# hamorrar/juicefs

Hardware: AMD Instinct MI355X
Metric: sealed+checksummed GB/s, 4 MiB blocks (higher is better)
Workload: dtype u8; 1 GPU; 64.0 GiB device-resident batch of 4 MiB blocks per GPU, aes256gcm seal + CRC32C full; blocks_per_gpu=16384, resident_blocks_per_gpu=16384, block_bytes=4194304, algo=aes256gcm, mode=seal, aes_kernel=ttable, engine=one process per GPU, parallelism=block-sharded x1, no collective

## Files before the change

juicefs_amd/csrc/jfsx_gcm.hip:

```cpp

#include "jfsx_dev.h"

#define JFSX_HD __device__ __forceinline__
#define BS3(a, b, c, tt) __builtin_amdgcn_bitop3_b32((a), (b), (c), (tt))
#define PERM(hi, lo, sel) __builtin_amdgcn_perm((hi), (lo), (sel))
#define OPAQUE(x)                                 \
    do {                                          \
        (x) = __builtin_amdgcn_readfirstlane(x);  \
        asm volatile("" : "+s"(x));               \
    } while (0)
#include "jfsx_aes_bs.h"

namespace jfsx {

constexpr int kAeadNt = 3;
constexpr uint32_t kLdsCrc = 0;
constexpr uint32_t kLdsTT = 20480;
constexpr uint32_t kLdsGh = 24576;
constexpr uint32_t kLdsAesOff = 24576;
constexpr uint32_t kLdsAes = 65536 + kLdsAesOff;
constexpr uint32_t kLdsBasis = kLdsAes + 65536;
constexpr uint32_t kLdsSegRaw = kLdsBasis + 2048;
constexpr uint32_t kLdsSegFlag = kLdsSegRaw + 512;
constexpr uint32_t kLdsP = kLdsSegFlag + 512;
constexpr uint32_t kLdsBytes = kLdsP + 4096;

__device__ __forceinline__ uint32_t rotl8(uint32_t x) { return __builtin_amdgcn_alignbit(x, x, 24); }
__device__ __forceinline__ uint32_t xor3(uint32_t a, uint32_t b, uint32_t c) {
    return __builtin_amdgcn_bitop3_b32(a, b, c, 0x96);
}
__device__ __forceinline__ uint32_t rk_load(const uint32_t *rk, int i) {
    uint32_t k = rk[i];
    if (i >= 8 && i < 56) {
        k = (k >> 8) | (k << 24);
        OPAQUE(k);
    }
    return k;
}

#define AES_SEL(k) (0x0c020000u | ((4u + (k)) << 8))
#define TA(w, k) lds_u32(lds, __builtin_amdgcn_perm((w), loff, AES_SEL(k)) + kLdsAesOff)
#define TB(w, k) lds_u32(lds, __builtin_amdgcn_perm((w), loff, AES_SEL(k)) + (kLdsAesOff + 128u))

#define AES_COL(o, i0, i1, i2, i3, rkv) \
    o = xor3(TA(i0, 0), TB(i2, 2), rotl8(xor3(TA(i1, 1), TB(i3, 3), (rkv))));
#define AES_ROUND(o0, o1, o2, o3, i0, i1, i2, i3, r) \
    AES_COL(o0, i0, i1, i2, i3, rk[4 * (r) + 0])     \
    AES_COL(o1, i1, i2, i3, i0, rk[4 * (r) + 1])     \
    AES_COL(o2, i2, i3, i0, i1, rk[4 * (r) + 2])     \
    AES_COL(o3, i3, i0, i1, i2, rk[4 * (r) + 3])

#define AES_LAST(o, a, b, c, d, rkv)                                                             \
    o = __builtin_amdgcn_bitop3_b32(                                                             \
            __builtin_amdgcn_bitop3_b32(TB(a, 0), TA(b, 1), 0xffu, 0xe4) ,       \
            __builtin_amdgcn_bitop3_b32(TA(c, 2), TB(d, 3), 0x00ff0000u, 0xe4),                 \
            0x0000ffffu, 0xe4) ^ (rkv);

template <int NS>
__device__ __forceinline__ void aes_ctr_blocks(const char *lds, uint32_t loff, const uint32_t *rk, const uint32_t *k1,
                                               const uint32_t (&ctr)[NS], uint32_t (&ks)[NS][4]) {
    uint32_t a[NS][4], b[NS][4];
#pragma unroll
    for (int s = 0; s < NS; s++) {
        const uint32_t x3 = __builtin_bswap32(ctr[s]) ^ rk[3];
        a[s][0] = k1[0] ^ rotl8(TB(x3, 3));
        a[s][1] = k1[1] ^ TB(x3, 2);
        a[s][2] = k1[2] ^ rotl8(TA(x3, 1));
        a[s][3] = k1[3] ^ TA(x3, 0);
    }
#pragma unroll
    for (int r = 2; r <= 13; r += 2) {
#pragma unroll
        for (int s = 0; s < NS; s++) { AES_ROUND(b[s][0], b[s][1], b[s][2], b[s][3], a[s][0], a[s][1], a[s][2], a[s][3], r); }
#pragma unroll
        for (int s = 0; s < NS; s++) { AES_ROUND(a[s][0], a[s][1], a[s][2], a[s][3], b[s][0], b[s][1], b[s][2], b[s][3], r + 1); }
    }
#pragma unroll
    for (int s = 0; s < NS; s++) {
        AES_LAST(ks[s][0], a[s][0], a[s][1], a[s][2], a[s][3], rk[56]);
        AES_LAST(ks[s][1], a[s][1], a[s][2], a[s][3], a[s][0], rk[57]);
        AES_LAST(ks[s][2], a[s][2], a[s][3], a[s][0], a[s][1], rk[58]);
        AES_LAST(ks[s][3], a[s][3], a[s][0], a[s][1], a[s][2], rk[59]);
    }
}

__device__ __forceinline__ void aes_r2_uniform(const char *lds, uint32_t loff, const uint32_t *rk, const uint32_t *k1,
                                               uint32_t U, uint32_t (&u)[4]) {
    const uint32_t x3 = __builtin_bswap32(U << 8) ^ rk[3];
    const uint32_t a1 = k1[1] ^ TB(x3, 2);
    const uint32_t a2 = k1[2] ^ rotl8(TA(x3, 1));
    const uint32_t a3 = k1[3] ^ TA(x3, 0);
    u[0] = xor3(TB(a2, 2), rotl8(xor3(TA(a1, 1), TB(a3, 3), rk[8])), 0u);
    u[1] = xor3(TA(a1, 0), TB(a3, 2), rotl8(TA(a2, 1) ^ rk[9]));
    u[2] = xor3(TA(a2, 0), rotl8(xor3(TA(a3, 1), TB(a1, 3), rk[10])), 0u);
    u[3] = xor3(TA(a3, 0), TB(a1, 2), rotl8(TB(a2, 3) ^ rk[11]));
}

__device__ __forceinline__ uint4 aes_r2_entry(const char *lds, uint32_t loff, uint32_t rk3, uint32_t k10, uint32_t c) {
    const uint32_t x3 = (c << 24) ^ rk3;
    const uint32_t a0 = k10 ^ rotl8(TB(x3, 3));
    return make_uint4(TA(a0, 0), rotl8(TB(a0, 3)), TB(a0, 2), rotl8(TA(a0, 1)));
}

template <int I>
struct AesStep {
    static constexpr int value = I;
};
struct AesNoSide {
    template <int I>
    __device__ __forceinline__ void operator()(AesStep<I>) const {}
};
template <int NS, class Side = AesNoSide>
__device__ __forceinline__ void aes_ctr_blocks_u(const char *lds, uint32_t loff, const uint32_t *rk,
                                                 const uint32_t *k1, const uint32_t (&ctr)[NS],
                                                 const uint32_t (&u)[NS][4], const uint32_t (&du)[NS][4],
                                                 const uint32_t (&cym)[NS], uint32_t (&ks)[NS][4],
                                                 const Side &side = Side()) {
    uint32_t a[NS][4], b[NS][4];
#define UC(t, w) (__builtin_amdgcn_bitop3_b32((t), cym[s], du[s][w], 0x78) ^ u[s][w])
#pragma unroll
    for (int s = 0; s < NS; s++) {
        const uint4 pe = lds_u4(lds, ((ctr[s] << 4) & 0xff0u) + kLdsP);
        b[s][0] = UC(pe.x, 0);
        b[s][1] = UC(pe.y, 1);
        b[s][2] = UC(pe.z, 2);
        b[s][3] = UC(pe.w, 3);
    }
#undef UC
    side(AesStep<0>());
#pragma unroll
    for (int s = 0; s < NS; s++) { AES_ROUND(a[s][0], a[s][1], a[s][2], a[s][3], b[s][0], b[s][1], b[s][2], b[s][3], 3); }
    side(AesStep<1>());
#define JFSX_AES_PAIR(r)                                                                                                \
    _Pragma("unroll") for (int s = 0; s < NS; s++) {                                                                    \
        AES_ROUND(b[s][0], b[s][1], b[s][2], b[s][3], a[s][0], a[s][1], a[s][2], a[s][3], r);                           \
    }                                                                                                                   \
    side(AesStep<(r) - 2>());                                                                                           \
    _Pragma("unroll") for (int s = 0; s < NS; s++) {                                                                    \
        AES_ROUND(a[s][0], a[s][1], a[s][2], a[s][3], b[s][0], b[s][1], b[s][2], b[s][3], (r) + 1);                     \
    }                                                                                                                   \
    side(AesStep<(r) - 1>());
    JFSX_AES_PAIR(4)
    JFSX_AES_PAIR(6)
    JFSX_AES_PAIR(8)
    JFSX_AES_PAIR(10)
    JFSX_AES_PAIR(12)
#undef JFSX_AES_PAIR
#pragma unroll
    for (int s = 0; s < NS; s++) {
        AES_LAST(ks[s][0], a[s][0], a[s][1], a[s][2], a[s][3], 0u);
        AES_LAST(ks[s][1], a[s][1], a[s][2], a[s][3], a[s][0], 0u);
        AES_LAST(ks[s][2], a[s][2], a[s][3], a[s][0], a[s][1], 0u);
        AES_LAST(ks[s][3], a[s][3], a[s][0], a[s][1], a[s][2], 0u);
    }
}

struct GhLane {
    uint32_t sel[4];
    uint32_t off[4];
    bool r1, r2;
    uint32_t p1, p2;
};

__device__ __forceinline__ GhLane gh_lane(uint32_t lane) {
    GhLane g;
    const uint32_t q = lane & 15, k = q >> 2;
#pragma unroll
    for (int bb = 0; bb < 4; bb++) g.sel[bb] = 0x0c0c0000u | ((4u + ((bb + q) & 3)) << 8) | (uint32_t)bb;
#pragma unroll
    for (int dd = 0; dd < 4; dd++) {
        uint32_t o = 0;
#pragma unroll
        for (int bb = 0; bb < 4; bb++) {
            const uint32_t j = 4 * ((dd + k) & 3) + ((bb + q) & 3);
            o |= (j << 4) << (8 * bb);
        }
        g.off[dd] = o;
    }
    g.r1 = (k & 1) != 0;
    g.r2 = (k & 2) != 0;
    g.p1 = g.r1 ? 0x07060504u : 0x03020100u;
    g.p2 = g.r2 ? 0x07060504u : 0x03020100u;
    return g;
}

__device__ __forceinline__ void gh_rho(const uint32_t a[4], const GhLane &g, uint32_t R[4]) {
    uint32_t u[4];
#pragma unroll
    for (int i = 0; i < 4; i++) u[i] = PERM(a[(i + 2) & 3], a[i], g.p2);
#pragma unroll
    for (int i = 0; i < 4; i++) R[i] = PERM(u[(i + 1) & 3], u[i], g.p1);
}
__device__ __forceinline__ void gh_rho_inv(const uint32_t R[4], const GhLane &g, uint32_t a[4]) {
    uint32_t u[4];
#pragma unroll
    for (int i = 0; i < 4; i++) u[i] = g.r1 ? R[(i + 3) & 3] : R[i];
#pragma unroll
    for (int i = 0; i < 4; i++) a[i] = g.r2 ? u[(i + 2) & 3] : u[i];
}

__device__ __forceinline__ void ghash_step(const char *lds, uint32_t R[4], const GhLane &g, uint4 c) {
#if JFSX_GH8 == 4
    uint32_t S[4] = {c.x, c.y, c.z, c.w};
#pragma unroll
    for (int h = 0; h < 4; h++) {
        uint4 t[4];
#pragma unroll
        for (int q = 0; q < 4; q++) t[q] = lds_u4(lds, kLdsGh + __builtin_amdgcn_perm(R[h], g.off[h], g.sel[q]));
#define GX(f, i) S[i] = xor3(xor3(t[0].f, t[1].f, t[2].f), t[3].f, S[i])
        GX(x, 0); GX(y, 1); GX(z, 2); GX(w, 3);
#undef GX
        __builtin_amdgcn_sched_barrier(0);
    }
#elif JFSX_GH8
    uint32_t S[4] = {c.x, c.y, c.z, c.w};
#pragma unroll
    for (int h = 0; h < 2; h++) {
        uint4 t[8];
#pragma unroll
        for (int q = 0; q < 8; q++) {
            const int dd = 2 * h + (q >> 2), bb = q & 3;
            t[q] = lds_u4(lds, kLdsGh + __builtin_amdgcn_perm(R[dd], g.off[dd], g.sel[bb]));
        }
#define GX(f, i) S[i] = xor3(xor3(t[0].f, t[1].f, t[2].f), xor3(t[3].f, t[4].f, t[5].f), xor3(t[6].f, t[7].f, S[i]))
        GX(x, 0); GX(y, 1); GX(z, 2); GX(w, 3);
#undef GX
        __builtin_amdgcn_sched_barrier(0);
    }
#else
    uint4 t[16];
#pragma unroll
    for (int dd = 0; dd < 4; dd++)
#pragma unroll
        for (int bb = 0; bb < 4; bb++)
            t[4 * dd + bb] = lds_u4(lds, kLdsGh + __builtin_amdgcn_perm(R[dd], g.off[dd], g.sel[bb]));
#define GX(f, cf) xor3(xor3(xor3(t[0].f, t[1].f, t[2].f), xor3(t[3].f, t[4].f, t[5].f), xor3(t[6].f, t[7].f, t[8].f)), \
                       xor3(t[9].f, t[10].f, t[11].f), xor3(xor3(t[12].f, t[13].f, t[14].f), t[15].f, cf))
    const uint32_t S[4] = {GX(x, c.x), GX(y, c.y), GX(z, c.z), GX(w, c.w)};
#undef GX
#endif
    gh_rho(S, g, R);
}

struct Stream {
    uint64_t sub0, sub1;
    uint32_t acc[4];
    uint64_t jlast;
    bool has;
    uint32_t A, lend;
    uint64_t seg0;
};

__device__ __forceinline__ void crc_share(char *lds, uint32_t slot, uint32_t raw) {
    atomicXor(reinterpret_cast<uint32_t *>(lds + kLdsSegRaw) + slot, raw);
    reinterpret_cast<uint32_t *>(lds + kLdsSegFlag)[slot] = 1u;
}

template <int CRCMODE>
__device__ __forceinline__ void crc_segment_done(const BlkDev &blk, const DevTables &tab, uint32_t lane, uint32_t xl,
                                                 uint64_t seg0, uint32_t A, bool partial, char *lds, uint64_t c0) {
    const uint32_t raw = wave_xor(crc_mulmod(xl, A));
    if (lane == 0) {
        if (partial) {
            crc_share(lds, (uint32_t)((seg0 - c0) / kSeg), raw);
            return;
        }
        const uint32_t crc = ~(tab.crcx[96] ^ raw);
        const uint64_t si = seg0 / kSeg;
        if ((CRCMODE & 3) == 1)
            *reinterpret_cast<uint32_t *>(blk.crc + 4 * si) = __builtin_bswap32(crc);
        else
            blk.crc_calc[si] = crc;
    }
}

template <int CRCMODE>
__device__ __noinline__ void crc_segment_end(const BlkDev &blk, const DevTables &tab, uint32_t lane, uint32_t xl,
                                             uint64_t seg0, uint64_t seg1, uint32_t A, uint32_t lend,
                                             uint64_t tailRef, bool partial, char *lds, uint32_t slot) {
    const uint32_t Lseg = (uint32_t)(seg1 - seg0);
    uint32_t v;
    if (lend == 0) {
        const uint32_t sh = tailRef == seg1 ? xl : crc_mulmod(crc_xpow8_fast((uint32_t)(seg1 - tailRef), tab.crcx), xl);
        v = crc_mulmod(sh, A);
    } else {
        v = crc_mulmod(crc_xpow8_fast(Lseg - lend, tab.crcx), A);
    }
    const uint32_t raw = wave_xor(v);
    if (lane == 0) {
        if (partial) {
            crc_share(lds, slot, raw);
            return;
        }
        const uint32_t K = Lseg == (uint32_t)kSeg ? tab.crcx[96] : crc_mulmod(crc_xpow8_fast(Lseg, tab.crcx), 0xffffffffu);
        const uint32_t crc = ~(K ^ raw);
        const uint64_t si = seg0 / kSeg;
        if ((CRCMODE & 3) == 1)
            *reinterpret_cast<uint32_t *>(blk.crc + 4 * si) = __builtin_bswap32(crc);
        else
            blk.crc_calc[si] = crc;
    }
}

template <bool OPEN, int CRCMODE>
__device__ __noinline__ Stream row_generic(char *lds, uint32_t loff, const GhLane gl, const GcmSched *sch,
                                           const BlkDev blk, const DevTables tab, uint32_t lane, uint32_t xl, Stream st,
                                           uint64_t row, uint64_t c0, uint64_t c1) {
    uint32_t rk[60];
#pragma unroll
    for (int i = 0; i < 60; i++) rk[i] = rk_load(sch->rk, i);
    const uint32_t k1[4] = {sch->k1[0], sch->k1[1], sch->k1[2], sch->k1[3]};
    const uint64_t o = row + 16 * lane;
    const uint64_t end = st.sub1;
    const bool valid = o < end, full = o + 16 <= end;
    uint4 d = load_piece(blk.src, o, end);
    const uint32_t ctr[1] = {(uint32_t)((o >> 4) + 2)};
    uint32_t ks[1][4];
    aes_ctr_blocks<1>(lds, loff, rk, k1, ctr, ks);
    uint4 x = make_uint4(d.x ^ ks[0][0], d.y ^ ks[0][1], d.z ^ ks[0][2], d.w ^ ks[0][3]);
    uint4 c = OPEN ? d : x, p = OPEN ? x : d;
    if (!full) {
        const int nv = valid ? (int)(end - o) : 0;
        uint32_t m[4];
        for (int k = 0; k < 4; k++) {
            int bytes = nv - 4 * k;
            m[k] = bytes >= 4 ? 0xffffffffu : (bytes <= 0 ? 0u : ((1u << (8 * bytes)) - 1u));
        }
        c.x &= m[0]; c.y &= m[1]; c.z &= m[2]; c.w &= m[3];
        p.x &= m[0]; p.y &= m[1]; p.z &= m[2]; p.w &= m[3];
    }
    if (valid) store_piece(blk.dst, o, end, OPEN ? p : c);
    uint32_t t[4] = {st.acc[0], st.acc[1], st.acc[2], st.acc[3]};
    ghash_step(lds, t, gl, c);
    if (valid) {
        st.acc[0] = t[0]; st.acc[1] = t[1]; st.acc[2] = t[2]; st.acc[3] = t[3];
        st.jlast = o >> 4;
        st.has = true;
    }
    const uint4 cq = crc_src<CRCMODE>(c, p);
    if (CRCMODE) {
        if (full) {
            st.A = crc_piece<kLdsCrc>(lds, st.A, cq.x, cq.y, cq.z, cq.w);
            st.lend = (uint32_t)(o + 16 - st.seg0);
        } else if (valid) {
            const uint32_t pw[4] = {cq.x, cq.y, cq.z, cq.w};
            st.A = crc_partial<kLdsCrc>(lds, st.A, pw, (int)(end - o));
            st.lend = (uint32_t)(end - st.seg0);
        }
        const uint64_t seg1 = st.seg0 + kSeg < c1 ? st.seg0 + kSeg : c1;
        if (row + 1024 >= seg1) {
            crc_segment_end<CRCMODE>(blk, tab, lane, xl, st.seg0, seg1, st.A, st.lend, row, st.seg0 < st.sub0, lds,
                                     (uint32_t)((st.seg0 - c0) / kSeg));
            st.A = 0;
            st.lend = 0;
            st.seg0 = seg1;
        }
    }
    return st;
}

template <bool BS>
struct GcmShape {
    static constexpr uint32_t waves = BS ? 8u : (uint32_t)kWaves;
    static constexpr uint32_t threads = waves * 64u;
};

#ifdef JFSX_KS_PHASES
__device__ unsigned long long g_main_ts[8];
#define MAIN_STAMP(cond, i)                                                                  \
    do {                                                                                     \
        __syncthreads();                                                                     \
        if ((cond) && threadIdx.x == 0) g_main_ts[i] = __builtin_amdgcn_s_memrealtime(); \
    } while (0)
#else
#define MAIN_STAMP(cond, i) ((void)0)
#endif

#ifdef JFSX_ABLATE_TRACE
__device__ uint64_t g_wgtrace[4 * 65536];
#endif

template <bool OPEN, int CRCMODE, bool BS, int KL1>
__device__ __forceinline__ void gcm_task(char *lds, const Task task, const BlkDev *__restrict__ blks,
                                         const GcmSched *__restrict__ sched, uint32_t *__restrict__ partial,
                                         uint32_t *__restrict__ pexp, const DevTables &tab, uint32_t tid,
                                         uint32_t wave, uint32_t lane, uint32_t loff, const GhLane &gl, uint32_t xl) {
#ifdef JFSX_ABLATE_TRACE
    const uint64_t trace_t0 = __builtin_amdgcn_s_memrealtime();
#endif
    const BlkDev blk = blks[task.blk];
    const GcmSched *sch = sched + task.blk;
    if (tid < 128)
        reinterpret_cast<uint4 *>(lds + kLdsBasis)[tid] = reinterpret_cast<const uint4 *>(sch->basis)[tid];
    if (tid < 256) reinterpret_cast<uint32_t *>(lds + kLdsSegRaw)[tid] = 0u;
    if (wave < 4) {
        uint32_t c = (wave << 6) | lane;
        asm volatile("" : "+v"(c));
        reinterpret_cast<uint4 *>(lds + kLdsP)[c] = aes_r2_entry(lds, loff, sch->rk[3], sch->k1[0], c);
    }
    __syncthreads();
    {
        uint4 *lg = reinterpret_cast<uint4 *>(lds + kLdsGh);
        const uint4 *lb = reinterpret_cast<const uint4 *>(lds + kLdsBasis);
#ifdef JFSX_ABLATE_GHBUILD
        if (false)
#endif
        for (uint32_t u = tid; u < 1024; u += GcmShape<BS>::threads) {
            const uint32_t j = u & 15, blow = u >> 4;
            uint4 z = make_uint4(0, 0, 0, 0);
#pragma unroll
            for (int k = 2; k < 8; k++) {
                if ((blow >> (7 - k)) & 1) {
                    const uint4 v = lb[8 * j + k];
                    z.x ^= v.x; z.y ^= v.y; z.z ^= v.z; z.w ^= v.w;
                }
            }
            const uint4 h0 = lb[8 * j], h1 = lb[8 * j + 1];
            lg[(blow << 4) | j] = z;
            lg[((blow | 64) << 4) | j] = make_uint4(z.x ^ h1.x, z.y ^ h1.y, z.z ^ h1.z, z.w ^ h1.w);
            lg[((blow | 128) << 4) | j] = make_uint4(z.x ^ h0.x, z.y ^ h0.y, z.z ^ h0.z, z.w ^ h0.w);
            lg[((blow | 192) << 4) | j] =
                make_uint4(z.x ^ h0.x ^ h1.x, z.y ^ h0.y ^ h1.y, z.z ^ h0.z ^ h1.z, z.w ^ h0.w ^ h1.w);
        }
    }
    __syncthreads();

    const bool first_task = task.blk == 0 && task.c0 == 0;
    MAIN_STAMP(first_task, 2);
    const uint64_t c0 = task.c0, c1 = task.c1;
    const uint32_t nseg = (uint32_t)((c1 - c0 + kSeg - 1) / kSeg);
    constexpr uint32_t V = GcmShape<BS>::waves;

    constexpr bool kRowSplit = !BS;
    Stream st;
    if (kRowSplit) {
        const uint32_t npairs = (uint32_t)((c1 - c0 + 2047) / 2048);
        const uint32_t ra = 2 * (wave * npairs / V), rb = 2 * ((wave + 1) * npairs / V);
        st.sub0 = c0 + (uint64_t)ra * 1024;
        st.sub1 = rb > ra ? (c0 + (uint64_t)rb * 1024 < c1 ? c0 + (uint64_t)rb * 1024 : c1) : st.sub0;
    } else {
        const uint32_t sa = wave * nseg / V, sb = (wave + 1) * nseg / V;
        st.sub0 = c0 + (uint64_t)sa * kSeg;
        st.sub1 = sb > sa ? (c0 + (uint64_t)sb * kSeg < c1 ? c0 + (uint64_t)sb * kSeg : c1) : st.sub0;
    }
    st.acc[0] = st.acc[1] = st.acc[2] = st.acc[3] = 0;
    st.jlast = 0;
    st.has = false;
    st.A = 0;
    st.lend = 0;
    st.seg0 = c0 + (st.sub0 - c0) / kSeg * kSeg;
    const bool act = st.sub1 > st.sub0;
    const uint64_t fr = (st.sub1 - st.sub0) / 1024;
    const uint64_t rf = act ? fr : 0;
    const uint64_t ld0 = st.sub0;
    const uint8_t *src = blk.src;
    uint8_t *dst = blk.dst;
    const uint64_t lo = 16 * lane;

    uint64_t r0 = 0;
    if (BS && act && rf >= 32) {
        const uint64_t nfs = rf / 32;
        const uint32_t nrk[3] = {sch->c012[0], sch->c012[1], sch->c012[2]};
        const uint32_t rk3 = sch->rk[3];
        constexpr int PF = 4;
        uint4 pf[PF];
#pragma unroll
        for (int q = 0; q < PF; q++) pf[q] = ald16<kAeadNt>(src + ld0 + 1024 * q + lo);
        for (uint64_t sg = 0; sg < nfs; sg++) {
            const uint64_t base = ld0 + (uint64_t)kSeg * sg;
            uint32_t ks[128];
            jfsx_bs::ctr32(ks, nrk, rk3, (uint32_t)((base >> 4) + lane + 2),
                           [&](int r, int w) { return sch->bsu[r][w]; }, sch->r1c);
            const bool more = sg + 1 < nfs;
#pragma unroll
            for (int k = 0; k < 32; k++) {
                const uint4 d = pf[k % PF];
                const uint64_t o = base + 1024 * k + lo;
                if (k + PF < 32 || more) pf[k % PF] = ald16<kAeadNt>(src + o + 1024 * PF);
                const uint4 x = make_uint4(d.x ^ ks[k], d.y ^ ks[32 + k], d.z ^ ks[64 + k], d.w ^ ks[96 + k]);
                const uint4 c = OPEN ? d : x, p = OPEN ? x : d;
                ast16<kAeadNt>(dst + o, OPEN ? p : c);
                const uint4 cq = crc_src<CRCMODE>(c, p);
                ghash_step(lds, st.acc, gl, c);
                if (CRCMODE) st.A = crc_piece<kLdsCrc>(lds, st.A, cq.x, cq.y, cq.z, cq.w);
            }
            if (CRCMODE) {
                crc_segment_done<CRCMODE>(blk, tab, lane, xl, st.seg0, st.A, false, lds, c0);
                st.A = 0;
                st.seg0 += kSeg;
            }
        }
        r0 = 32 * nfs;
    }
    uint32_t rk[60];
#pragma unroll
    for (int i = 0; i < 60; i++) rk[i] = rk_load(sch->rk, i);
    uint32_t k1[4] = {sch->k1[0], sch->k1[1], sch->k1[2], sch->k1[3]};
    uint4 nxt = r0 < rf ? ald16<kAeadNt>(src + ld0 + 1024 * r0 + lo) : make_uint4(0, 0, 0, 0);
    constexpr int UR = 2;
    constexpr bool kL1 = KL1 > 0 && kRowSplit && CRCMODE != 0 && OPEN == ((CRCMODE & 4) != 0);
    auto xl_here = [&]() { return kL1 ? crc_xl(tab, lane) : xl; };
    static_assert(!kL1 || KL1 == 12, "B form: TT_4..15 are in the L1 image only");
    bool bform = false;
    if (act && rf >= r0 + UR) {
        uint4 nn[UR];
#pragma unroll
        for (int u = 0; u < UR; u++) nn[u] = ald16<kAeadNt>(src + ld0 + 1024 * (r0 + u) + lo);
        uint32_t uw[4] = {0, 0, 0, 0};
        uint32_t uw0 = 0;
        bool uwok = false;
        const uint32_t rb0 = (uint32_t)((ld0 - c0) >> 10) / 2u * 2u;
        const CrcL1Base l1g = kL1 ? crc_l1_base(crc_composed(tab)) : CrcL1Base{0, 0};
        for (; r0 + UR - 1 < rf; r0 += UR) {
            uint4 dd[UR];
#pragma unroll
            for (int u = 0; u < UR; u++) dd[u] = nn[u];
            const uint64_t o0 = ld0 + 1024 * r0 + lo;
            if (!kL1 && r0 + 2 * UR - 1 < rf) {
#pragma unroll
                for (int u = 0; u < UR; u++) nn[u] = ald16<kAeadNt>(src + o0 + 1024 * (UR + u));
            }
            constexpr int LG = kL1 ? JFSX_CRC_L1LG : 1, LLAG = JFSX_CRC_L1LAG, LSTEPS = kL1 ? UR * KL1 / LG : 0;
            static_assert(!kL1 || (KL1 % LG == 0 && LSTEPS + LLAG <= 12),
                          "the gathers, their folds and the prefetch must fit the 12 round groups");
            uint32_t crcL[UR], lv[LSTEPS ? LSTEPS : 1][LG];
#pragma unroll
            for (int u = 0; u < UR; u++) crcL[u] = 0;
            const bool pre = r0 + 2 * UR - 1 < rf;
            auto side = [&](auto step) {
                if constexpr (kL1) {
                    constexpr int S = decltype(step)::value;
                    __builtin_amdgcn_sched_barrier(0);
                    if constexpr (S >= LLAG && S - LLAG < LSTEPS) {
                        constexpr int F = S - LLAG;
                        uint32_t t = crcL[F % UR];
#pragma unroll
                        for (int j = 0; j + 1 < LG; j += 2) t = xor3(t, lv[F][j], lv[F][j + 1]);
                        if (LG & 1) t ^= lv[F][LG - 1];
                        crcL[F % UR] = t;
                    }
                    if constexpr (S < LSTEPS) {
                        crc_l1_issue<S, LG, UR>(l1g, dd, lv[S]);
                    } else if constexpr (S == LSTEPS) {
                        if (pre) {
#pragma unroll
                            for (int u = 0; u < UR; u++) nn[u] = ald16<kAeadNt>(src + o0 + 1024 * (UR + u));
                        }
                    }
                    __builtin_amdgcn_sched_barrier(0);
                }
            };
            uint32_t ctrs[UR];
#pragma unroll
            for (int u = 0; u < UR; u++) ctrs[u] = (uint32_t)((o0 >> 4) + 2 + 64 * u);
            uint32_t ks2[UR][4];
            {
                uint32_t C = (uint32_t)(((ld0 + 1024 * r0) >> 4) + 2);
                OPAQUE(C);
                if (!uwok || (C >> 8) < uw0 || ((C + 64u * UR + 63u) >> 8) - uw0 > 63u) {
                    uw0 = C >> 8;
                    aes_r2_uniform(lds, loff, rk, k1, uw0 + lane, uw);
                    uwok = true;
                }
                uint32_t u2[UR][4], d2[UR][4], cym[UR];
#pragma unroll
                for (int u = 0; u < UR; u++) {
                    const uint32_t Cr = C + 64u * u;
                    const uint32_t i0 = (Cr >> 8) - uw0;
                    cym[u] = (uint32_t)__builtin_amdgcn_sbfe((int)((Cr & 255u) + lane), 8, 1);
#pragma unroll
                    for (int k = 0; k < 4; k++) {
                        u2[u][k] = __builtin_amdgcn_readlane(uw[k], i0);
                        d2[u][k] = u2[u][k] ^ __builtin_amdgcn_readlane(uw[k], i0 + 1);
                    }
                }
                aes_ctr_blocks_u<UR>(lds, loff, rk, k1, ctrs, u2, d2, cym, ks2, side);
            }
#pragma unroll
            for (int u = 0; u < UR; u++) {
                const uint64_t o = o0 + 1024 * u;
                const uint4 x = make_uint4(xor3(dd[u].x, ks2[u][0], rk[56]), xor3(dd[u].y, ks2[u][1], rk[57]),
                                           xor3(dd[u].z, ks2[u][2], rk[58]), xor3(dd[u].w, ks2[u][3], rk[59]));
                const uint4 c = OPEN ? dd[u] : x, p = OPEN ? x : dd[u];
                ast16<kAeadNt>(dst + o, OPEN ? p : c);
                const uint4 cq = crc_src<CRCMODE>(c, p);
                ghash_step(lds, st.acc, gl, c);
                if constexpr (kL1)
                    st.A = crc_piece_b<kLdsTT>(lds, st.A, cq.x, crcL[u]);
                else if (CRCMODE)
                    st.A = crc_piece<kLdsCrc>(lds, st.A, cq.x, cq.y, cq.z, cq.w);
                if (CRCMODE && ((rb0 + (uint32_t)r0 + u) & 31) == 31) {
                    crc_segment_done<CRCMODE>(blk, tab, lane, kL1 ? crc_xlb(tab, lane) : xl, st.seg0,
                                              st.A, st.seg0 < st.sub0, lds, c0);
                    st.A = 0;
                    st.seg0 += kSeg;
                }
            }
        }
        if (r0 < rf) nxt = ald16<kAeadNt>(src + ld0 + 1024 * r0 + lo);
        if constexpr (kL1) bform = ((rb0 + (uint32_t)r0) & 31) != 0;
    }
    for (uint64_t r = r0; r < rf; r++) {
        uint4 d[1];
        uint32_t ctr[1];
#pragma unroll
        for (int s = 0; s < 1; s++) {
            d[s] = nxt;
            const uint64_t o = ld0 + 1024 * r + lo;
            if (r + 1 < rf) nxt = ald16<kAeadNt>(src + o + 1024);
            ctr[s] = (uint32_t)((o >> 4) + 2);
        }
        uint32_t ks[1][4];
        aes_ctr_blocks<1>(lds, loff, rk, k1, ctr, ks);
#pragma unroll
        for (int s = 0; s < 1; s++) {
            if (!act) continue;
            const uint64_t o = st.sub0 + 1024 * r + lo;
            const uint4 x = make_uint4(d[s].x ^ ks[s][0], d[s].y ^ ks[s][1], d[s].z ^ ks[s][2], d[s].w ^ ks[s][3]);
            const uint4 c = OPEN ? d[s] : x, p = OPEN ? x : d[s];
            ast16<kAeadNt>(dst + o, OPEN ? p : c);
            const uint4 cq = crc_src<CRCMODE>(c, p);
            ghash_step(lds, st.acc, gl, c);
            if constexpr (kL1) {
                const uint32_t sh = bform ? st.A : crc_shift1008<kLdsCrc>(lds, st.A);
                st.A = crc_piece<kLdsCrc, -1>(lds, sh, cq.x, cq.y, cq.z, cq.w);
            } else if (CRCMODE)
                st.A = crc_piece<kLdsCrc>(lds, st.A, cq.x, cq.y, cq.z, cq.w);
        }
        if constexpr (kL1) bform = false;
        if (CRCMODE && ((uint32_t)((ld0 - c0) >> 10) + (uint32_t)r & 31) == 31) {
            if (act) {
                crc_segment_done<CRCMODE>(blk, tab, lane, xl_here(), st.seg0, st.A, st.seg0 < st.sub0, lds, c0);
                st.A = 0;
                st.seg0 += kSeg;
            }
        }
    }
#pragma unroll
    for (int s = 0; s < 1; s++) {
        if (rf && act) {
            st.has = true;
            st.jlast = (st.sub0 + 1024 * (rf - 1) + lo) >> 4;
        }
        const uint64_t tailRef = st.sub0 + 1024 * rf;
        if constexpr (kL1) {
            if (bform && tailRef < st.sub1) {
                st.A = crc_mulmod(crc_xlb(tab, 63), st.A);
                bform = false;
            }
        }
        for (uint64_t row = tailRef; row < st.sub1; row += 1024)
            st = row_generic<OPEN, CRCMODE>(lds, loff, gl, sch, blk, tab, lane, xl_here(), st, row, c0, c1);
        if (CRCMODE && act && st.seg0 < st.sub1) {
            const uint64_t seg1 = st.seg0 + kSeg < c1 ? st.seg0 + kSeg : c1;
            uint32_t xle;
            if constexpr (kL1)
                xle = bform ? crc_xlb(tab, lane) : crc_xl(tab, lane);
            else
                xle = xl;
            crc_segment_end<CRCMODE>(blk, tab, lane, xle, st.seg0, seg1, st.A, st.lend, tailRef,
                                     st.seg0 < st.sub0 || st.sub1 < seg1, lds, (uint32_t)((st.seg0 - c0) / kSeg));
            st.seg0 = st.sub1;
        }
    }

    MAIN_STAMP(first_task, 3);
    const uint64_t nblk = (blk.len + 15) >> 4;
#pragma unroll
    for (int s = 0; s < 1; s++) {
        const uint64_t wend = (st.sub1 + 15) >> 4;
        g128 z = {{0, 0, 0, 0}};
        if (st.has && st.sub1 > st.sub0) {
            const uint32_t e = (uint32_t)(wend + 1 - st.jlast);
            uint32_t a[4];
            gh_rho_inv(st.acc, gl, a);
#ifdef JFSX_ABLATE_LIFT
            z = g_from_mem(a);
#else
            z = g_mul_ct_call(g_from_mem(a), g_from_mem(sch->hpow[e]));
#endif
        }
        uint32_t zm[4];
        g_to_mem(z, zm);
        for (int k = 0; k < 4; k++) zm[k] = wave_xor(zm[k]);
        if (lane == 0) {
            const uint32_t slot = task.slot0 + wave;
            partial[4 * slot + 0] = zm[0];
            partial[4 * slot + 1] = zm[1];
            partial[4 * slot + 2] = zm[2];
            partial[4 * slot + 3] = zm[3];
            pexp[slot] = (uint32_t)(nblk - wend);
            for (uint32_t u = task.slot0 + V + wave; u < task.slot0 + kSlotsPerTask; u += V) {
                partial[4 * u + 0] = partial[4 * u + 1] = partial[4 * u + 2] = partial[4 * u + 3] = 0;
                pexp[u] = 0;
            }
        }
    }

#ifdef JFSX_ABLATE_TRACE
    __syncthreads();
    if (tid == 0 && task.trace < 65536) {
        uint32_t hw, xcc;
        asm volatile("s_getreg_b32 %0, hwreg(HW_REG_HW_ID)" : "=s"(hw));
        asm volatile("s_getreg_b32 %0, hwreg(HW_REG_XCC_ID)" : "=s"(xcc));
        g_wgtrace[4 * task.trace + 0] = trace_t0;
        g_wgtrace[4 * task.trace + 1] = __builtin_amdgcn_s_memrealtime();
        g_wgtrace[4 * task.trace + 2] = hw | ((uint64_t)xcc << 32);
        g_wgtrace[4 * task.trace + 3] = task.c1 - task.c0;
    }
#endif
    MAIN_STAMP(first_task, 4);
    if (CRCMODE && kRowSplit) {
        __syncthreads();
        if (wave == 0) {
            const uint32_t *raw = reinterpret_cast<const uint32_t *>(lds + kLdsSegRaw);
            const uint32_t *flag = reinterpret_cast<const uint32_t *>(lds + kLdsSegFlag);
            for (uint32_t k = lane; k < nseg; k += 64) {
                if (!flag[k]) continue;
                const uint64_t s0 = c0 + (uint64_t)k * kSeg;
                const uint32_t Lseg = (uint32_t)((s0 + kSeg < c1 ? s0 + kSeg : c1) - s0);
                const uint32_t K = Lseg == (uint32_t)kSeg ? tab.crcx[96]
                                                          : crc_mulmod(crc_xpow8_fast(Lseg, tab.crcx), 0xffffffffu);
                const uint32_t crc = ~(K ^ raw[k]);
                const uint64_t si = s0 / kSeg;
                if ((CRCMODE & 3) == 1)
                    *reinterpret_cast<uint32_t *>(blk.crc + 4 * si) = __builtin_bswap32(crc);
                else
                    blk.crc_calc[si] = crc;
            }
        }
    }
    MAIN_STAMP(first_task, 5);
}

template <bool OPEN, int CRCMODE, bool BS, int KL1 = 0>
__global__ __launch_bounds__(GcmShape<BS>::threads) void gcm_main_k(const Task *__restrict__ tasks, uint32_t ntasks,
                                                       uint32_t *__restrict__ queue,
                                                       const BlkDev *__restrict__ blks,
                                                       const GcmSched *__restrict__ sched,
                                                       uint32_t *__restrict__ partial, uint32_t *__restrict__ pexp,
                                                       DevTables tab) {
    __shared__ __attribute__((aligned(16))) char lds[kLdsBytes];
    __shared__ uint32_t s_task;
    const uint32_t tid = threadIdx.x;
#ifdef JFSX_KS_PHASES
    const unsigned long long t_start = __builtin_amdgcn_s_memrealtime();
#endif
    {
        const uint4 *ga = reinterpret_cast<const uint4 *>(tab.aes);
        uint4 *la = reinterpret_cast<uint4 *>(lds + kLdsAes);
        for (uint32_t i = tid; i < 4096; i += GcmShape<BS>::threads) la[i] = ga[i];
        if (CRCMODE) {
            const uint4 *gc = reinterpret_cast<const uint4 *>(tab.crc);
            uint4 *lc = reinterpret_cast<uint4 *>(lds + kLdsCrc);
            for (uint32_t i = tid; i < 1280; i += GcmShape<BS>::threads) lc[i] = gc[i];
        }
        if (KL1) {
            const uint4 *gt = reinterpret_cast<const uint4 *>(crc_composed(tab));
            if (tid < 256) reinterpret_cast<uint4 *>(lds + kLdsTT)[tid] = gt[tid];
        }
    }
#ifdef JFSX_KS_PHASES
    __syncthreads();
    const unsigned long long t_staged = __builtin_amdgcn_s_memrealtime();
    if (tid == 0 && tasks[0].blk == 0 && blockIdx.x == 0) {
        g_main_ts[0] = t_start;
        g_main_ts[1] = t_staged;
    }
#endif
    const uint32_t wave = __builtin_amdgcn_readfirstlane(tid >> 6), lane = tid & 63;
    const uint32_t loff = ((lane & 31) << 2) | 0x00010000u;
    const GhLane gl = gh_lane(lane);
    const uint32_t xl = CRCMODE && !KL1 ? tab.crcx[lane] : 0u;
    if (tid == 0) s_task = atomicAdd(queue, 1u);
    for (;;) {
        __syncthreads();
        const uint32_t ti = __builtin_amdgcn_readfirstlane(s_task);
        if (ti >= ntasks) break;
        __syncthreads();
        if (tid == 0) s_task = atomicAdd(queue, 1u);
        gcm_task<OPEN, CRCMODE, BS, KL1>(lds, tasks[ti], blks, sched, partial, pexp, tab, tid, wave, lane, loff, gl,
                                         xl);
    }
}

__device__ __forceinline__ uint32_t gT0(const uint32_t *aes, uint32_t x) { return aes[2 * x]; }
__device__ __forceinline__ uint32_t gT2(const uint32_t *aes, uint32_t x) { return aes[2 * x + 1]; }
__device__ __forceinline__ uint32_t gS(const uint32_t *aes, uint32_t x) { return (aes[2 * x] >> 8) & 0xffu; }

__device__ uint32_t gcol(const uint32_t *aes, uint32_t a, uint32_t b, uint32_t c, uint32_t d) {
    return gT0(aes, a & 0xff) ^ rotl8(gT0(aes, (b >> 8) & 0xff)) ^ gT2(aes, (c >> 16) & 0xff) ^
           rotl8(gT2(aes, d >> 24));
}

__device__ void aes_enc_global(const uint32_t *aes, const uint32_t *rk, const uint32_t in[4], uint32_t out[4]) {
    uint32_t s[4], t[4];
#pragma unroll
    for (int c = 0; c < 4; c++) s[c] = in[c] ^ rk[c];
    for (int r = 1; r < 14; r++) {
#pragma unroll
        for (int c = 0; c < 4; c++) t[c] = gcol(aes, s[c], s[(c + 1) & 3], s[(c + 2) & 3], s[(c + 3) & 3]) ^ rk[4 * r + c];
#pragma unroll
        for (int c = 0; c < 4; c++) s[c] = t[c];
    }
#pragma unroll
    for (int c = 0; c < 4; c++) {
        uint32_t a = s[c], b = s[(c + 1) & 3], cc = s[(c + 2) & 3], d = s[(c + 3) & 3];
        out[c] = (gS(aes, a & 0xff) | (gS(aes, (b >> 8) & 0xff) << 8) | (gS(aes, (cc >> 16) & 0xff) << 16) |
                  (gS(aes, d >> 24) << 24)) ^ rk[56 + c];
    }
}

#ifdef JFSX_KS_PHASES
__device__ unsigned long long g_ks_ts[16];
#define KS_STAMP(i)                                                          \
    do {                                                                     \
        __syncthreads();                                                     \
        if (blockIdx.x == 0 && threadIdx.x == 0) g_ks_ts[i] = __builtin_amdgcn_s_memrealtime(); \
    } while (0)
#else
#define KS_STAMP(i) ((void)0)
#endif

template <int S>
__device__ __forceinline__ g128 g_mulxs(g128 v) {
    constexpr int q = S / 32, r = S % 32;
    uint32_t a[4], b[4], t[4];
#pragma unroll
    for (int k = 0; k < 4; k++) a[k] = v.w[(k - q + 4) & 3];
#pragma unroll
    for (int k = 0; k < 4; k++) b[k] = r ? __builtin_amdgcn_alignbit(a[(k + 3) & 3], a[k], r) : a[k];
#pragma unroll
    for (int k = 0; k < 4; k++) {
        const int top = S - 32 * k;
        t[k] = top >= 32 ? b[k] : top > 0 ? b[k] & ~(0xffffffffu >> top) : 0u;
    }
    g128 z;
#pragma unroll
    for (int k = 0; k < 4; k++) {
        const uint32_t p = k ? t[k - 1] : 0u;
        z.w[k] = b[k] ^ __builtin_amdgcn_alignbit(p, t[k], 1) ^ __builtin_amdgcn_alignbit(p, t[k], 2) ^
                 __builtin_amdgcn_alignbit(p, t[k], 7);
    }
    return z;
}

__device__ __forceinline__ g128 g_mul_xpow(g128 v, uint32_t i) {
    g128 u;
#define JFSX_XPOW_STEP(K)                                       \
    u = g_mulxs<(1 << K)>(v);                                   \
    if ((i >> K) & 1u) v = u;
    JFSX_XPOW_STEP(0)
    JFSX_XPOW_STEP(1)
    JFSX_XPOW_STEP(2)
    JFSX_XPOW_STEP(3)
    JFSX_XPOW_STEP(4)
    JFSX_XPOW_STEP(5)
    JFSX_XPOW_STEP(6)
#undef JFSX_XPOW_STEP
    return v;
}

__global__ __launch_bounds__(64) void gcm_keysetup_k(const KeyIn *__restrict__ keys, const BlkDev *__restrict__ blks,
                                                    GcmSched *__restrict__ sched, const uint32_t *__restrict__ gtab,
                                                    int need_bs) {
    const uint32_t b = blockIdx.x, lane = threadIdx.x;
    KS_STAMP(0);
    GcmSched *sc = sched + b;
    const KeyIn k = keys[b];
    __shared__ uint32_t aes[512];
    for (uint32_t x = lane; x < 256; x += 64) {
        aes[2 * x] = gtab[x * 64];
        aes[2 * x + 1] = gtab[x * 64 + 32];
    }
    __syncthreads();
    KS_STAMP(1);
    __shared__ uint32_t sw[60];
    if (lane == 0) {
        uint32_t e[60];
#pragma unroll
        for (int i = 0; i < 8; i++) e[i] = k.key[i];
        uint32_t rcon = 1;
#pragma unroll
        for (int i = 8; i < 60; i++) {
            uint32_t t = e[i - 1];
            if ((i & 7) == 0) {
                t = (t >> 8) | (t << 24);
                t = gS(aes, t & 0xff) | (gS(aes, (t >> 8) & 0xff) << 8) | (gS(aes, (t >> 16) & 0xff) << 16) |
                    (gS(aes, t >> 24) << 24);
                t ^= rcon;
                rcon <<= 1;
            } else if ((i & 7) == 4) {
                t = gS(aes, t & 0xff) | (gS(aes, (t >> 8) & 0xff) << 8) | (gS(aes, (t >> 16) & 0xff) << 16) |
                    (gS(aes, t >> 24) << 24);
            }
            e[i] = e[i - 8] ^ t;
        }
#pragma unroll
        for (int i = 0; i < 60; i++) sw[i] = e[i];
    }
    __syncthreads();
    KS_STAMP(2);
    const uint32_t *w = sw;
    if (lane < 60) sc->rk[lane] = sw[lane];
    if (need_bs) {
        const uint32_t my = lane < 56 ? jfsx_bs::round_mask_word(sw, 1 + (int)(lane >> 2), (int)(lane & 3)) : 0u;
        if (lane < 56) sc->bsu[1 + (lane >> 2)][lane & 3] = my;
        const uint32_t x0w[3] = {k.nonce[0] ^ w[0], k.nonce[1] ^ w[1], k.nonce[2] ^ w[2]};
        const uint32_t sb = lane < 12 ? jfsx_bs::sbox_byte((x0w[lane >> 2] >> (8 * (lane & 3))) & 0xffu) : 0u;
        uint32_t sbn[12];
        for (int i = 0; i < 12; i++) sbn[i] = (uint32_t)__shfl(sb, i, 64);
        const uint32_t u1[4] = {(uint32_t)__shfl(my, 0, 64), (uint32_t)__shfl(my, 1, 64), (uint32_t)__shfl(my, 2, 64),
                                (uint32_t)__shfl(my, 3, 64)};
        if (lane < 4) sc->r1c[lane] = jfsx_bs::round1_const(sbn, u1, (int)lane);
    }
    const uint32_t x0 = k.nonce[0] ^ w[0], x1 = k.nonce[1] ^ w[1], x2 = k.nonce[2] ^ w[2];
    if (lane == 0) {
        sc->c012[0] = x0; sc->c012[1] = x1; sc->c012[2] = x2;
        sc->k1[0] = w[4] ^ gT0(aes, x0 & 0xff) ^ rotl8(gT0(aes, (x1 >> 8) & 0xff)) ^ gT2(aes, (x2 >> 16) & 0xff);
        sc->k1[1] = w[5] ^ gT0(aes, x1 & 0xff) ^ rotl8(gT0(aes, (x2 >> 8) & 0xff)) ^ rotl8(gT2(aes, x0 >> 24));
        sc->k1[2] = w[6] ^ gT0(aes, x2 & 0xff) ^ gT2(aes, (x0 >> 16) & 0xff) ^ rotl8(gT2(aes, x1 >> 24));
        sc->k1[3] = w[7] ^ rotl8(gT0(aes, (x0 >> 8) & 0xff)) ^ gT2(aes, (x1 >> 16) & 0xff) ^ rotl8(gT2(aes, x2 >> 24));
    }
    KS_STAMP(3);
    uint32_t in[4], o[4], Hm[4], EJ0[4];
    {
        const bool j = lane >= 32;
        in[0] = j ? k.nonce[0] : 0u;
        in[1] = j ? k.nonce[1] : 0u;
        in[2] = j ? k.nonce[2] : 0u;
        in[3] = j ? 0x01000000u : 0u;
        aes_enc_global(aes, w, in, o);
#pragma unroll
        for (int q = 0; q < 4; q++) {
            Hm[q] = (uint32_t)__shfl(o[q], 0, 64);
            EJ0[q] = (uint32_t)__shfl(o[q], 32, 64);
        }
    }
    const g128 H = g_from_mem(Hm);
    KS_STAMP(4);
    uint32_t nsq;
    {
        const uint64_t nb16 = (blks[b].len + 15) / 16 + 2;
        const uint32_t bits = 64u - (uint32_t)__builtin_clzll(nb16);
        nsq = bits + 1 < 8 ? 8u : bits + 1 > 32 ? 32u : bits + 1;
    }
    __shared__ g128 hs[8];
    g128 g = H;
    for (uint32_t i = 0; i < nsq; i++) {
        if (i < 8 && lane == 0) hs[i] = g;
        if (lane == i) {
            uint32_t m[4];
            g_to_mem(g, m);
            for (int q = 0; q < 4; q++) sc->h2k[i][q] = m[q];
        }
        g = g_sqr(g);
    }
    __syncthreads();
    KS_STAMP(5);
    {
        g128 z = {{0x80000000u, 0, 0, 0}};
        for (int q = 0; q < 6; q++) {
            const g128 m = g_mul_ct_call(z, hs[q]);
            if ((lane >> q) & 1) z = m;
        }
        const g128 z64 = g_mul_ct_call(z, hs[6]);
        uint32_t m[4];
        g_to_mem(z, m);
        for (int q = 0; q < 4; q++) sc->hpow[lane][q] = m[q];
        if (lane < 4) {
            g_to_mem(z64, m);
            for (int q = 0; q < 4; q++) sc->hpow[64 + lane][q] = m[q];
        }
    }
    KS_STAMP(6);
    {
        const g128 v = g_mul_xpow(hs[6], lane), v64 = g_mulxs<64>(v);
        uint32_t m[4];
        g_to_mem(v, m);
        for (int q = 0; q < 4; q++) sc->basis[lane][q] = m[q];
        g_to_mem(v64, m);
        for (int q = 0; q < 4; q++) sc->basis[64 + lane][q] = m[q];
    }
    KS_STAMP(7);
    {
        const uint64_t bits = blks[b].len * 8;
        g128 L = {{0, 0, (uint32_t)(bits >> 32), (uint32_t)bits}};
        const g128 LH = g_mul_ct_call(L, H);
        if (lane == 0) {
            uint32_t m[4];
            g_to_mem(LH, m);
            for (int q = 0; q < 4; q++) sc->init[q] = m[q] ^ EJ0[q];
        }
    }
    KS_STAMP(8);
}

#ifdef JFSX_KS_PHASES
extern "C" int jfsx_debug_main_phases(unsigned long long *out) {
    return hipMemcpyFromSymbol(out, HIP_SYMBOL(g_main_ts), sizeof(g_main_ts)) == hipSuccess ? 0 : -1;
}
extern "C" int jfsx_debug_ks_phases(unsigned long long *out) {
    return hipMemcpyFromSymbol(out, HIP_SYMBOL(g_ks_ts), sizeof(g_ks_ts)) == hipSuccess ? 0 : -1;
}
#endif

template <bool OPEN, int CRCMODE, int TH>
__global__ __launch_bounds__(TH) void gcm_finalize_k(const BlkDev *__restrict__ blks, const GcmSched *__restrict__ sched,
                                                      const uint32_t *__restrict__ partial,
                                                      const uint32_t *__restrict__ pexp, BlkOut *__restrict__ out) {
    const uint32_t b = blockIdx.x, tid = threadIdx.x, lane = tid & 63, wave = tid >> 6, nthr = blockDim.x;
    const uint32_t nw = nthr >> 6;
    __shared__ uint32_t sor[16];
    __shared__ uint32_t sred[16][4];
    __shared__ uint32_t h2k[32][4];
    const BlkDev blk = blks[b];
    const GcmSched *sc = sched + b;
    for (uint32_t i = tid; i < 128; i += nthr) h2k[i >> 2][i & 3] = sc->h2k[i >> 2][i & 3];
    __syncthreads();
    uint32_t acc[4] = {0, 0, 0, 0};
    for (uint32_t base = 0; base < blk.nslots; base += nthr) {
        const uint32_t s = base + tid;
        uint32_t m[4] = {0, 0, 0, 0}, e = 0;
        if (s < blk.nslots) {
            const uint32_t slot = blk.slot0 + s;
            for (int q = 0; q < 4; q++) m[q] = partial[4 * slot + q];
            if (m[0] | m[1] | m[2] | m[3]) e = pexp[slot];
        }
        uint32_t eo = e;
        for (int off = 32; off > 0; off >>= 1) eo |= __shfl_xor(eo, off, 64);
        if (lane == 0) sor[wave] = eo;
        __syncthreads();
        eo = 0;
        for (uint32_t w = 0; w < nw; w++) eo |= sor[w];
        g128 z = g_from_mem(m);
        for (int k = 0; k < 32 && (eo >> k); k++) {
            if (!((eo >> k) & 1u)) continue;
            const g128 zk = g_mul_ct_call(z, g_from_mem(h2k[k]));
            if ((e >> k) & 1u) z = zk;
        }
        g_to_mem(z, m);
        for (int q = 0; q < 4; q++) acc[q] ^= m[q];
        __syncthreads();
    }
    for (int q = 0; q < 4; q++) acc[q] = wave_xor(acc[q]);
    if (lane == 0)
        for (int q = 0; q < 4; q++) sred[wave][q] = acc[q];
    __syncthreads();
    if (wave) return;
    for (int q = 0; q < 4; q++) {
        uint32_t t = sc->init[q];
        for (uint32_t w = 0; w < nw; w++) t ^= sred[w][q];
        acc[q] = t;
    }
    BlkOut o;
    o.status = JFSX_OK;
    o.bad_seg = -1;
    o.got = o.expect = 0;
    for (int q = 0; q < 4; q++) o.tag[q] = acc[q];
    if (OPEN) {
        const uint32_t *t = reinterpret_cast<const uint32_t *>(blk.tag_in);
        uint32_t d = 0;
        for (int q = 0; q < 4; q++) d |= acc[q] ^ t[q];
        if (d) o.status = JFSX_ETAG;
    }
    if ((CRCMODE & 3) == 2) {
        crc_verify_block(blk, o, lane);
        if (o.bad_seg >= 0 && o.status == JFSX_OK) o.status = JFSX_ECRC;
    }
    if (lane == 0) out[b] = o;
}

void launch_gcm_keysetup(hipStream_t s, int n, const KeyIn *keys, const BlkDev *blks, GcmSched *sched, DevTables t,
                         bool bitslice) {
    if (n > 0)
        hipLaunchKernelGGL(gcm_keysetup_k, dim3(n), dim3(64), 0, s, keys, blks, sched, t.aes,
                           (int)bitslice);
}

void launch_gcm_main(hipStream_t s, int ntasks, int ncu, uint32_t *queue, bool open, int crc_mode, bool bitslice,
                     const Task *tasks, const BlkDev *blks, const GcmSched *sched, uint32_t *partial, uint32_t *pexp,
                     DevTables t, bool crc_l1) {
    if (ntasks <= 0) return;
    const unsigned grid = (unsigned)(ntasks < ncu ? ntasks : ncu);
#define L(O, C)                                                                                              \
    do {                                                                                                     \
        if (bitslice)                                                                                        \
            hipLaunchKernelGGL((gcm_main_k<O, C, true>), dim3(grid), dim3(GcmShape<true>::threads), 0, s, tasks, \
                               (uint32_t)ntasks, queue, blks, sched, partial, pexp, t);                      \
        else if (crc_l1 && (C) != 0 && (O) == (((C) & 4) != 0))                                              \
            hipLaunchKernelGGL((gcm_main_k<O, C, false, ((C) != 0 && (O) == (((C) & 4) != 0)) ? JFSX_CRC_L1K : 0>), \
                               dim3(grid), dim3(GcmShape<false>::threads), 0, s, tasks, (uint32_t)ntasks, queue, blks, \
                               sched, partial, pexp, t);                                                     \
        else                                                                                                 \
            hipLaunchKernelGGL((gcm_main_k<O, C, false>), dim3(grid), dim3(GcmShape<false>::threads), 0, s,  \
                               tasks, (uint32_t)ntasks, queue, blks, sched, partial, pexp, t);               \
    } while (0)
    switch ((open ? 8 : 0) | crc_mode) {
        case 8: L(true, 0); break;
        case 9: L(true, 1); break;
        case 10: L(true, 2); break;
        case 13: L(true, 5); break;
        case 14: L(true, 6); break;
        case 0: L(false, 0); break;
        case 1: L(false, 1); break;
        case 2: L(false, 2); break;
        case 5: L(false, 5); break;
        case 6: L(false, 6); break;
    }
#undef L
}

void launch_gcm_finalize(hipStream_t s, int n, bool open, int crc_mode, const BlkDev *blks, const GcmSched *sched,
                         const uint32_t *partial, const uint32_t *pexp, BlkOut *out, uint32_t max_slots) {
    if (n <= 0) return;
    const uint32_t th = max_slots <= 64 ? 64u : max_slots >= 1024 ? 1024u : (max_slots + 63) / 64 * 64;
#define L(O, C)                                                                                          \
    do {                                                                                                 \
        if (th == 64)                                                                                    \
            hipLaunchKernelGGL((gcm_finalize_k<O, C, 64>), dim3(n), dim3(64), 0, s, blks, sched, partial, pexp, out); \
        else                                                                                             \
            hipLaunchKernelGGL((gcm_finalize_k<O, C, 1024>), dim3(n), dim3(th), 0, s, blks, sched, partial, pexp, out); \
    } while (0)
    if (open) {
        if ((crc_mode & 3) == 2) L(true, 2); else L(true, 0);
    } else {
        if ((crc_mode & 3) == 2) L(false, 2); else L(false, 0);
    }
#undef L
}

}

#ifdef JFSX_ABLATE_TRACE
extern "C" __attribute__((visibility("default"))) int jfsx_debug_wgtrace(uint64_t *out, int n) {
    if (n > 65536) n = 65536;
    return hipMemcpyFromSymbol(out, HIP_SYMBOL(jfsx::g_wgtrace), 32 * (size_t)n) == hipSuccess ? 0 : -5;
}
#endif
```

Baseline: 917.6 GB/s.

## Add four-row periodic AES-CTR path using fixed per-lane round-2 table offsets

For the non-bitsliced path, rows are now processed four at a time, aligned so that the low counter byte follows a fixed per-lane pattern. The round-2 table entry can then be read at a constant per-lane LDS offset instead of being recomputed from the counter each row. The round-2 table gets two extra wrap-around entries, and the uniform carry correction is needed only on the last quarter. CRC segment-boundary checks are restricted to the final row of each pair or quad. This trims per-row address arithmetic and branch checks, at the cost of more code, a larger unrolled body and possible extra register pressure.

```diff
diff --git a/juicefs_amd/csrc/jfsx_gcm.hip b/juicefs_amd/csrc/jfsx_gcm.hip
--- a/juicefs_amd/csrc/jfsx_gcm.hip
+++ b/juicefs_amd/csrc/jfsx_gcm.hip
@@ -23,7 +23,7 @@
 constexpr uint32_t kLdsSegRaw = kLdsBasis + 2048;
 constexpr uint32_t kLdsSegFlag = kLdsSegRaw + 512;
 constexpr uint32_t kLdsP = kLdsSegFlag + 512;
-constexpr uint32_t kLdsBytes = kLdsP + 4096;
+constexpr uint32_t kLdsBytes = kLdsP + 4096 + 32;
 
 __device__ __forceinline__ uint32_t rotl8(uint32_t x) { return __builtin_amdgcn_alignbit(x, x, 24); }
 __device__ __forceinline__ uint32_t xor3(uint32_t a, uint32_t b, uint32_t c) {
@@ -110,23 +110,10 @@
     template <int I>
     __device__ __forceinline__ void operator()(AesStep<I>) const {}
 };
-template <int NS, class Side = AesNoSide>
-__device__ __forceinline__ void aes_ctr_blocks_u(const char *lds, uint32_t loff, const uint32_t *rk,
-                                                 const uint32_t *k1, const uint32_t (&ctr)[NS],
-                                                 const uint32_t (&u)[NS][4], const uint32_t (&du)[NS][4],
-                                                 const uint32_t (&cym)[NS], uint32_t (&ks)[NS][4],
-                                                 const Side &side = Side()) {
-    uint32_t a[NS][4], b[NS][4];
-#define UC(t, w) (__builtin_amdgcn_bitop3_b32((t), cym[s], du[s][w], 0x78) ^ u[s][w])
-#pragma unroll
-    for (int s = 0; s < NS; s++) {
-        const uint4 pe = lds_u4(lds, ((ctr[s] << 4) & 0xff0u) + kLdsP);
-        b[s][0] = UC(pe.x, 0);
-        b[s][1] = UC(pe.y, 1);
-        b[s][2] = UC(pe.z, 2);
-        b[s][3] = UC(pe.w, 3);
-    }
-#undef UC
+template <int NS, class Side>
+__device__ __forceinline__ void aes_rounds_3_14(const char *lds, uint32_t loff, const uint32_t *rk,
+                                                uint32_t (&b)[NS][4], uint32_t (&ks)[NS][4], const Side &side) {
+    uint32_t a[NS][4];
     side(AesStep<0>());
 #pragma unroll
     for (int s = 0; s < NS; s++) { AES_ROUND(a[s][0], a[s][1], a[s][2], a[s][3], b[s][0], b[s][1], b[s][2], b[s][3], 3); }
@@ -155,6 +142,42 @@
     }
 }
 
+template <int NS, class Side = AesNoSide>
+__device__ __forceinline__ void aes_ctr_blocks_u(const char *lds, uint32_t loff, const uint32_t *rk,
+                                                 const uint32_t *k1, const uint32_t (&ctr)[NS],
+                                                 const uint32_t (&u)[NS][4], const uint32_t (&du)[NS][4],
+                                                 const uint32_t (&cym)[NS], uint32_t (&ks)[NS][4],
+                                                 const Side &side = Side()) {
+    uint32_t b[NS][4];
+#define UC(t, w) (__builtin_amdgcn_bitop3_b32((t), cym[s], du[s][w], 0x78) ^ u[s][w])
+#pragma unroll
+    for (int s = 0; s < NS; s++) {
+        const uint4 pe = lds_u4(lds, ((ctr[s] << 4) & 0xff0u) + kLdsP);
+        b[s][0] = UC(pe.x, 0);
+        b[s][1] = UC(pe.y, 1);
+        b[s][2] = UC(pe.z, 2);
+        b[s][3] = UC(pe.w, 3);
+    }
+#undef UC
+    aes_rounds_3_14<NS>(lds, loff, rk, b, ks, side);
+}
+
+template <int Q, class Side>
+__device__ __forceinline__ void aes_ctr_blocks_p(const char *lds, uint32_t loff, const uint32_t *rk, uint32_t pb,
+                                                 const uint32_t (&u)[4], const uint32_t (&du)[4], uint32_t cy3,
+                                                 uint32_t (&ks)[2][4], const Side &side) {
+    uint32_t b[2][4];
+#pragma unroll
+    for (int s = 0; s < 2; s++) {
+        const uint4 pe = lds_u4(lds, pb + 1024u * (Q + s));
+        const uint32_t t[4] = {pe.x, pe.y, pe.z, pe.w};
+#pragma unroll
+        for (int w = 0; w < 4; w++)
+            b[s][w] = Q + s == 3 ? __builtin_amdgcn_bitop3_b32(t[w], cy3, du[w], 0x78) ^ u[w] : t[w] ^ u[w];
+    }
+    aes_rounds_3_14<2>(lds, loff, rk, b, ks, side);
+}
+
 struct GhLane {
     uint32_t sel[4];
     uint32_t off[4];
@@ -396,7 +419,11 @@
     if (wave < 4) {
         uint32_t c = (wave << 6) | lane;
         asm volatile("" : "+v"(c));
-        reinterpret_cast<uint4 *>(lds + kLdsP)[c] = aes_r2_entry(lds, loff, sch->rk[3], sch->k1[0], c);
+        const uint4 e = aes_r2_entry(lds, loff, sch->rk[3], sch->k1[0], c);
+        reinterpret_cast<uint4 *>(lds + kLdsP)[c] = e;
+        if constexpr (!BS) {
+            if (c < 2) reinterpret_cast<uint4 *>(lds + kLdsP)[256 + c] = e;
+        }
     }
     __syncthreads();
     {
@@ -499,6 +526,7 @@
     uint4 nxt = r0 < rf ? ald16<kAeadNt>(src + ld0 + 1024 * r0 + lo) : make_uint4(0, 0, 0, 0);
     constexpr int UR = 2;
     constexpr bool kL1 = KL1 > 0 && kRowSplit && CRCMODE != 0 && OPEN == ((CRCMODE & 4) != 0);
+    constexpr bool kPeriod = !BS;
     auto xl_here = [&]() { return kL1 ? crc_xl(tab, lane) : xl; };
     static_assert(!kL1 || KL1 == 12, "B form: TT_4..15 are in the L1 image only");
     bool bform = false;
@@ -511,7 +539,7 @@
         bool uwok = false;
         const uint32_t rb0 = (uint32_t)((ld0 - c0) >> 10) / 2u * 2u;
         const CrcL1Base l1g = kL1 ? crc_l1_base(crc_composed(tab)) : CrcL1Base{0, 0};
-        for (; r0 + UR - 1 < rf; r0 += UR) {
+        auto two_rows = [&]() __attribute__((always_inline)) {
             uint4 dd[UR];
 #pragma unroll
             for (int u = 0; u < UR; u++) dd[u] = nn[u];
@@ -589,14 +617,110 @@
                     st.A = crc_piece_b<kLdsTT>(lds, st.A, cq.x, crcL[u]);
                 else if (CRCMODE)
                     st.A = crc_piece<kLdsCrc>(lds, st.A, cq.x, cq.y, cq.z, cq.w);
-                if (CRCMODE && ((rb0 + (uint32_t)r0 + u) & 31) == 31) {
+                if (CRCMODE && (!kPeriod || u == UR - 1) && ((rb0 + (uint32_t)r0 + u) & 31) == 31) {
                     crc_segment_done<CRCMODE>(blk, tab, lane, kL1 ? crc_xlb(tab, lane) : xl, st.seg0,
                                               st.A, st.seg0 < st.sub0, lds, c0);
                     st.A = 0;
                     st.seg0 += kSeg;
                 }
             }
-        }
+        };
+        {
+            if constexpr (kPeriod) {
+                if ((((uint32_t)((ld0 + 1024 * r0) >> 4) + 2u) & 255u) != 2u) {
+                    two_rows();
+                    r0 += UR;
+                }
+                {
+                    for (; r0 + 3 < rf; r0 += 4) {
+                        const uint64_t o0 = ld0 + 1024 * r0 + lo;
+                        auto half = [&](auto q, const uint4(&dd)[UR], uint4(&pf)[UR], const bool pre, const uint32_t pb,
+                                        const uint32_t(&up)[4], const uint32_t(&dp)[4],
+                                        const uint32_t cy3) __attribute__((always_inline)) {
+                            constexpr int Q = decltype(q)::value;
+                            if (!kL1 && pre) {
+#pragma unroll
+                                for (int u = 0; u < UR; u++) pf[u] = ald16<kAeadNt>(src + o0 + 1024 * (Q + UR + u));
+                            }
+                            constexpr int LG = kL1 ? JFSX_CRC_L1LG : 1, LLAG = JFSX_CRC_L1LAG,
+                                          LSTEPS = kL1 ? UR * KL1 / LG : 0;
+                            uint32_t crcL[UR], lv[LSTEPS ? LSTEPS : 1][LG];
+#pragma unroll
+                            for (int u = 0; u < UR; u++) crcL[u] = 0;
+                            auto side = [&](auto step) {
+                                if constexpr (kL1) {
+                                    constexpr int S = decltype(step)::value;
+                                    __builtin_amdgcn_sched_barrier(0);
+                                    if constexpr (S >= LLAG && S - LLAG < LSTEPS) {
+                                        constexpr int F = S - LLAG;
+                                        uint32_t t = crcL[F % UR];
+#pragma unroll
+                                        for (int j = 0; j + 1 < LG; j += 2) t = xor3(t, lv[F][j], lv[F][j + 1]);
+                                        if (LG & 1) t ^= lv[F][LG - 1];
+                                        crcL[F % UR] = t;
+                                    }
+                                    if constexpr (S < LSTEPS) {
+                                        crc_l1_issue<S, LG, UR>(l1g, dd, lv[S]);
+                                    } else if constexpr (S == LSTEPS) {
+                                        if (pre) {
+#pragma unroll
+                                            for (int u = 0; u < UR; u++)
+                                                pf[u] = ald16<kAeadNt>(src + o0 + 1024 * (Q + UR + u));
+                                        }
+                                    }
+                                    __builtin_amdgcn_sched_barrier(0);
+                                }
+                            };
+                            uint32_t ks2[UR][4];
+                            aes_ctr_blocks_p<Q>(lds, loff, rk, pb, up, dp, cy3, ks2, side);
+#pragma unroll
+                            for (int u = 0; u < UR; u++) {
+                                const uint64_t o = o0 + 1024 * (Q + u);
+                                const uint4 x =
+                                    make_uint4(xor3(dd[u].x, ks2[u][0], rk[56]), xor3(dd[u].y, ks2[u][1], rk[57]),
+                                               xor3(dd[u].z, ks2[u][2], rk[58]), xor3(dd[u].w, ks2[u][3], rk[59]));
+                                const uint4 c = OPEN ? dd[u] : x, p = OPEN ? x : dd[u];
+                                ast16<kAeadNt>(dst + o, OPEN ? p : c);
+                                const uint4 cq = crc_src<CRCMODE>(c, p);
+                                ghash_step(lds, st.acc, gl, c);
+                                if constexpr (kL1)
+                                    st.A = crc_piece_b<kLdsTT>(lds, st.A, cq.x, crcL[u]);
+                                else if (CRCMODE)
+                                    st.A = crc_piece<kLdsCrc>(lds, st.A, cq.x, cq.y, cq.z, cq.w);
+                                if (CRCMODE && Q + u == 3 && ((rb0 + (uint32_t)r0 + 3u) & 31) == 31) {
+                                    crc_segment_done<CRCMODE>(blk, tab, lane, kL1 ? crc_xlb(tab, lane) : xl, st.seg0,
+                                                              st.A, st.seg0 < st.sub0, lds, c0);
+                                    st.A = 0;
+                                    st.seg0 += kSeg;
+                                }
+                            }
+                            asm volatile("" : "+v"(st.A), "+v"(st.acc[0]), "+v"(st.acc[1]), "+v"(st.acc[2]), "+v"(st.acc[3]));
+                        };
+                        uint32_t U = (uint32_t)((ld0 + 1024 * r0) >> 12);
+                        OPAQUE(U);
+                        if (!uwok || U < uw0 || U + 1u - uw0 > 63u) {
+                            uw0 = U;
+                            aes_r2_uniform(lds, loff, rk, k1, uw0 + lane, uw);
+                            uwok = true;
+                        }
+                        const uint32_t i0 = U - uw0;
+                        uint32_t up[4], dp[4];
+#pragma unroll
+                        for (int k = 0; k < 4; k++) up[k] = __builtin_amdgcn_readlane(uw[k], i0);
+                        uint32_t pl = lane;
+                        asm volatile("" : "+v"(pl));
+                        const uint32_t pb = (pl << 4) + (kLdsP + 32u);
+                        const uint32_t cy3 = pl >= 62u ? ~0u : 0u;
+                        uint4 mm[UR];
+                        half(AesStep<0>(), nn, mm, true, pb, up, up, 0u);
+#pragma unroll
+                        for (int k = 0; k < 4; k++) dp[k] = up[k] ^ __builtin_amdgcn_readlane(uw[k], i0 + 1);
+                        half(AesStep<2>(), mm, nn, r0 + 5 < rf, pb, up, dp, cy3);
+                    }
+                }
+            }
+        }
+        for (; r0 + UR - 1 < rf; r0 += UR) two_rows();
         if (r0 < rf) nxt = ald16<kAeadNt>(src + ld0 + 1024 * r0 + lo);
         if constexpr (kL1) bform = ((rb0 + (uint32_t)r0) & 31) != 0;
     }
```

Result: faster. 933.9 GB/s, median of 6 (+1.8%).
